# abalakrishna123/recovery-rl

Measured on AMD Instinct MI355X. Metric: env-steps/sec + SAC grad-steps/sec, Navigation1 4096 envs, 1/2/4/8 GPU, higher is better.
Workload: dtype f32

## Files before the change

### include/rrl_hip.h

```cpp
#ifndef RRL_HIP_H
#define RRL_HIP_H

#include <stdint.h>

#ifdef __cplusplus
extern "C" {
#endif

#define RRL_OK 0
#define RRL_EINVAL (-1)
#define RRL_ELAUNCH (-2)
#define RRL_ECAPTURE (-5)
#define RRL_EPLANS (-6)
#define RRL_ERANGE (-3)

enum { RRL_ENV_NAV1 = 0, RRL_ENV_NAV2 = 1, RRL_ENV_MAZE = 2 };

enum {
    RRL_STREAM_STEP = 0,
    RRL_STREAM_RESET = 1,
    RRL_STREAM_OFFLINE = 2,
    RRL_STREAM_SAMPLE = 3,
    RRL_STREAM_SAMPLE_NEG = 4,
    RRL_STREAM_CEM = 5,
// ... 301 lines not shown
int rrl_adam_step_multi(int n_seg, const rrl_adam_seg_t* segs, float lr, float beta1, float beta2, float eps,
                        void* stream);
#define RRL_ADAM_MAX_DUALS 4
typedef struct {
    float *log_p, *exp_avg, *exp_avg_sq, *step;
    float* value;
    const float* stat;
    float eps_safe;
    float lr;
    const float* loss_in;
    float* loss_out;
    float f_loss;
} rrl_dual_t;
int rrl_adam_step_multi_duals(int n_seg, const rrl_adam_seg_t* segs, int n_dual, const rrl_dual_t* duals, float lr,
                              float beta1, float beta2, float eps, void* stream);
int rrl_w2_pack(int G, int H, const float* W2, float* W2p, void* stream);
int rrl_normal_fill(long long n_pairs, uint64_t seed, uint64_t counter, uint64_t* counter_dev, uint64_t counter_inc,
                    float* out, void* stream);
int rrl_recovery_select(int N, const float* z, float eps_safe, const float* task_action, int ld_task,
                        const float* rec_action, float* real_action, uint8_t* recovery, float* task_out,
                        void* stream);

#define RRL_EPLOG_I32 6
typedef struct {
    int32_t* rec_i32;
    double* rec_f64;
    int64_t cap;
    int64_t* state;
} rrl_episode_log_t;

int rrl_episode_log_append(int64_t n, const float* reward, const uint8_t* constraint, const uint8_t* success,
                           const uint8_t* ep_done, const uint8_t* recovery, int32_t* ep_len, double* ep_ret,
                           int32_t* ep_viol, int32_t* ep_rec, const rrl_episode_log_t* log, void* stream);

typedef struct {
    int hq, he, n_nets;
    const float *q_w1, *q_b1, *q_w2, *q_b2, *q_w3, *q_b3;
    const float *e_w0, *e_b0, *e_w1, *e_b1, *e_w2, *e_b2, *e_w3, *e_b3;
    const float *inputs_mu, *inputs_sigma, *max_logvar, *min_logvar;
} rrl_plan_weights_t;

int rrl_plan_supported(int hq, int he, int n_nets, int npart, int d_obs, int d_act);
long long rrl_plan_pack_floats(int hq, int he, int n_nets);
long long rrl_plan_scratch_floats(int n_nets, long long M, int pop);
int rrl_plan_pack(const rrl_plan_weights_t* w, int f16x3, float* packed, void* stream);
typedef struct {
    const float* packed;
    int hq, he, n_nets, npart;
    int f16x3;
    long long M;
    const int32_t* m_dev;
    int pop, plan_hor;
    const float *cur_obs, *ac_seqs, *noise;
    uint64_t seed, counter;
    uint64_t* counter_dev;
    uint64_t counter_inc;
    float *scratch, *costs;
} rrl_plan_cost_t;
int rrl_plan_cost(const rrl_plan_cost_t* a, void* stream);

typedef struct {
    int n_nets, d_in, hidden, d_out;
    float *w0, *b0, *w1, *b1, *w2, *b2, *w3, *b3, *max_logvar, *min_logvar;
    const float *mu, *sigma;
    float *g_w0, *g_b0, *g_w1, *g_b1, *g_w2, *g_b2, *g_w3, *g_b3, *g_max_logvar, *g_min_logvar, *g_logvar_part;
    float *g2_w0, *g2_b0, *g2_w1, *g2_b1, *g2_w2, *g2_b2, *g2_w3, *g2_b3;
// ... 166 lines not shown
```

### recovery_rl_amd/_lib.py

```python
import ctypes as C
import os
import subprocess

_HERE = os.path.dirname(os.path.abspath(__file__))
CSRC = os.path.join(_HERE, "csrc")
SO_PATH = os.environ.get("RRL_HIP_LIB") or os.path.join(CSRC, "librrl_hip.so")
INCLUDE = os.path.join(os.path.dirname(_HERE), "include")

HIP_SOURCES = ["nav_kernels.hip", "replay_kernels.hip", "maze_kernels.hip", "cem_kernels.hip",
               "mlp_kernels.hip", "mlp_fwd_kernels.hip", "update_kernels.hip", "log_kernels.hip", "plan_kernels.hip", "ens_train_kernels.hip",
               "ens_train_big_kernels.hip", "sqrl_kernels.hip", "qsample_kernels.hip", "eval_kernels.hip"]
HIPCC_FLAGS = ["--offload-arch=gfx950", "-O3", "-std=c++17", "-fPIC", "-shared",
               "-ffp-contract=off", "-Wall", "-Wno-unused-function",
               "-Wno-bitwise-instead-of-logical"]

SOURCE_FLAGS = {
    "nav_kernels.hip": ["-mllvm", "-amdgpu-atomic-optimizer-strategy=None"],
    "maze_kernels.hip": ["-mllvm", "-amdgpu-atomic-optimizer-strategy=None"],
    "update_kernels.hip": ["-mllvm", "-amdgpu-atomic-optimizer-strategy=None"],
}

EXPORTS = [
    "rrl_abi_version", "rrl_last_hip_error", "rrl_counter_add",
    "rrl_nav_step", "rrl_nav_step_compact", "rrl_nav_reset", "rrl_nav_rollout", "rrl_nav_offline_rollouts",
    "rrl_nav_offline",
    "rrl_maze_step", "rrl_maze_reset", "rrl_maze_offline",
    "rrl_replay_push", "rrl_sample_multi", "rrl_draw_select", "rrl_mlp3_forward_riders",
    "rrl_nav_step_push_x", "rrl_maze_step_push_x",
    "rrl_sample_multi_packed", "rrl_pack_clear", "rrl_mlp3_forward_multi_packed", "rrl_mlp_head_backward_multi_packed",
    "rrl_mlp_hidden_backward_multi_packed", "rrl_mlp_backward_pair_multi_packed", "rrl_adam_step_multi_packed", "rrl_nav_step_push_packed",
    "rrl_maze_step_push_packed",
    "rrl_adam_step_multi_duals_packed", "rrl_rcpo_penalty_packed", "rrl_policy_heads_fwd_multi_packed",
    "rrl_cem_sample", "rrl_cem_update", "rrl_cem_begin", "rrl_cem_finish",
    "rrl_gemm_f32", "rrl_mlp3_forward", "rrl_mlp3_is_split",
    "rrl_mlp3_forward_multi", "rrl_mlp_head_backward_multi", "rrl_mlp_hidden_backward_multi",
    "rrl_mlp_input_backward_multi", "rrl_mlp_backward_pair_multi", "rrl_policy_heads_fwd_multi",
    "rrl_loss_dout", "rrl_rcpo_penalty", "rrl_adam_step_multi_duals",
    "rrl_adam_step_multi", "rrl_w2_pack", "rrl_normal_fill", "rrl_recovery_select", "rrl_episode_log_append",
    "rrl_plan_supported", "rrl_plan_pack_floats", "rrl_plan_scratch_floats", "rrl_plan_pack", "rrl_plan_cost",
    "rrl_ens_train_supported", "rrl_ens_scratch_floats", "rrl_ens_train_grad", "rrl_ens_train_epoch",
    "rrl_ens_train_big_supported", "rrl_ens_big_scratch_floats", "rrl_ens_train_grad_big", "rrl_ens_train_epoch_big",
    "rrl_sqrl_scratch_floats", "rrl_sqrl_act", "rrl_sqrl_act_packed",
    "rrl_qsample_scratch_floats", "rrl_qsample_act", "rrl_qsample_act_gated", "rrl_qsample_act_packed",
    "rrl_eval_rollout", "rrl_eval_rollout_packed", "rrl_eval_rollout_maze", "rrl_eval_rollout_maze_packed",
    "rrl_eval_rollout_qs", "rrl_eval_rollout_qs_packed",
    "rrl_eval_rollout_sqrl", "rrl_eval_rollout_sqrl_packed",
]

class RRLError(RuntimeError):
    pass


def _sources():
    return [os.path.join(CSRC, f) for f in HIP_SOURCES if os.path.exists(os.path.join(CSRC, f))]


def _stale():
    if not os.path.exists(SO_PATH):
        return True
    t = os.path.getmtime(SO_PATH)
    deps = _sources() + [os.path.join(CSRC, f) for f in os.listdir(CSRC) if f.endswith(".hpp")]
    deps.append(os.path.join(INCLUDE, "rrl_hip.h"))
    return any(os.path.getmtime(d) > t for d in deps)


_FLAG_PROBES = {}


def flags_supported(hipcc, flags):
    key = (hipcc,) + tuple(flags)
    if key not in _FLAG_PROBES:
# ... 25 lines not shown
        extra = SOURCE_FLAGS.get(os.path.basename(src), [])
        if extra and not flags_supported(hipcc, extra):
            extra = []
        cmd = [hipcc] + compile_flags + extra + ["-I", INCLUDE, "-c", "-o", obj, src]
        if verbose:
            print(" ".join(cmd))
        subprocess.check_call(cmd)
        return obj

    with ThreadPoolExecutor(max_workers=jobs or min(4, os.cpu_count() or 1)) as pool:
        objs = list(pool.map(compile_one, _sources()))
    cmd = [hipcc, "--offload-arch=gfx950", "-fPIC", "-shared", "-o", SO_PATH] + objs
    if verbose:
        print(" ".join(cmd))
    subprocess.check_call(cmd)
    return SO_PATH


class rrl_replay_t(C.Structure):
    _fields_ = [("s", C.c_void_p), ("a", C.c_void_p), ("r", C.c_void_p), ("s2", C.c_void_p),
                ("m", C.c_void_p), ("cap", C.c_int64), ("state", C.c_void_p),
                ("pos_cnt", C.c_void_p), ("flags", C.c_int32), ("pinned", C.c_int64)]


REPLAY_CLAMP_STRATIFIED = 1
DRAW_UNIFORM, DRAW_STRATIFIED, DRAW_DEMO_SHARE = 0, 1, 2


class rrl_episode_log_t(C.Structure):
    _fields_ = [("rec_i32", C.c_void_p), ("rec_f64", C.c_void_p), ("cap", C.c_int64), ("state", C.c_void_p)]


EPLOG_I32 = 6
ADAM_MAX_SEGS = 12
LOSS_SAC_CRITIC, LOSS_SAC_POLICY, LOSS_QRISK_CRITIC, LOSS_QRISK_POLICY, LOSS_GAUSS_HEAD, LOSS_STOCH_HEAD, LOSS_DGD_QRISK = range(7)
ADAM_MAX_DUALS = 4


class rrl_ens_t(C.Structure):
    _fields_ = [("n_nets", C.c_int), ("d_in", C.c_int), ("hidden", C.c_int), ("d_out", C.c_int)] + [
        (name, C.c_void_p) for name in ("w0", "b0", "w1", "b1", "w2", "b2", "w3", "b3", "max_logvar", "min_logvar",
                                        "mu", "sigma", "g_w0", "g_b0", "g_w1", "g_b1", "g_w2", "g_b2", "g_w3", "g_b3",
                                        "g_max_logvar", "g_min_logvar", "g_logvar_part", "g2_w0", "g2_b0", "g2_w1",
                                        "g2_b1", "g2_w2", "g2_b2", "g2_w3", "g2_b3", "loss_part")]


class rrl_loss_t(C.Structure):
    _fields_ = [("kind", C.c_int), ("n_part", C.c_int), ("part_stride", C.c_longlong), ("out", C.c_void_p),
                ("out_t", C.c_void_p), ("v0", C.c_void_p), ("v1", C.c_void_p), ("v2", C.c_void_p),
                ("v3", C.c_void_p), ("alpha", C.c_void_p), ("f0", C.c_float), ("ld", C.c_int),
                ("n_heads", C.c_int), ("head_stride", C.c_longlong), ("d_action", C.c_void_p),
                ("loss", C.c_void_p), ("da_parts", C.c_int), ("da_part_stride", C.c_longlong), ("da_group", C.c_int)]


HEAD_GAUSS, HEAD_STOCH = 0, 1


class rrl_policy_head_t(C.Structure):
    _fields_ = [("kind", C.c_int), ("B", C.c_int), ("head", C.c_void_p), ("n_part", C.c_int),
                ("part_stride", C.c_longlong), ("eps", C.c_void_p), ("scale", C.c_void_p), ("bias", C.c_void_p),
                ("action", C.c_void_p), ("ld_action", C.c_int), ("logp", C.c_void_p), ("mean_out", C.c_void_p),
                ("obs_in", C.c_void_p), ("obs_out", C.c_void_p), ("log_std", C.c_void_p), ("min_log_std", C.c_float)]


class rrl_step_push_t(C.Structure):
    _fields_ = [("n", C.c_int64), ("pos", C.c_void_p), ("t", C.c_void_p), ("status", C.c_void_p), ("obs", C.c_void_p),
# ... 232 lines not shown
        "rrl_normal_fill": (ci, [ll, u64, u64, vp, u64, vp, vp]),
        "rrl_recovery_select": (ci, [ci, vp, f32, vp, ci, vp, vp, vp, vp, vp]),
        "rrl_plan_supported": (ci, [ci, ci, ci, ci, ci, ci]),
        "rrl_plan_pack_floats": (ll, [ci, ci, ci]),
        "rrl_plan_scratch_floats": (ll, [ci, ll, ci]),
        "rrl_plan_pack": (ci, [C.POINTER(rrl_plan_weights_t), ci, vp, vp]),
        "rrl_plan_cost": (ci, [C.POINTER(rrl_plan_cost_t), vp]),
        "rrl_ens_train_supported": (ci, [ci, ci, ci, ci]),
        "rrl_ens_scratch_floats": (ll, [ci]),
        "rrl_ens_train_epoch": (ci, [C.POINTER(rrl_ens_t), ci, C.POINTER(rrl_adam_seg_t), f32, f32, f32, f32, vp, vp,
                                     vp, ll, ll, ci, vp, vp, vp]),
        "rrl_ens_train_grad": (ci, [C.POINTER(rrl_ens_t), ci, vp, vp, vp, ll, vp, vp, vp]),
        "rrl_ens_train_big_supported": (ci, [ci, ci, ci]),
        "rrl_ens_big_scratch_floats": (ll, [ci, ll]),
        "rrl_ens_train_grad_big": (ci, [C.POINTER(rrl_ens_t), ll, vp, vp, vp, ll, vp, vp, vp]),
        "rrl_ens_train_epoch_big": (ci, [C.POINTER(rrl_ens_t), ci, C.POINTER(rrl_adam_seg_t), f32, f32, f32, f32, vp, vp,
                                         vp, ll, ll, ll, vp, vp, vp]),
        "rrl_sqrl_scratch_floats": (ll, [ll, ci]),
        "rrl_sqrl_act": (ci, [C.POINTER(rrl_sqrl_act_t), vp]),
        "rrl_sqrl_act_packed": (ci, [ci, C.POINTER(rrl_sqrl_act_t), vp]),
        "rrl_qsample_scratch_floats": (ll, [ll, ci]),
        "rrl_qsample_act": (ci, [C.POINTER(rrl_qsample_act_t), vp]),
        "rrl_qsample_act_gated": (ci, [C.POINTER(rrl_qsample_act_t), C.POINTER(rrl_qsample_gate_t), vp]),
        "rrl_qsample_act_packed": (ci, [ci, C.POINTER(rrl_qsample_act_t), C.POINTER(rrl_qsample_gate_t), vp]),
        "rrl_eval_rollout": (ci, [C.POINTER(rrl_eval_rollout_t), vp]),
        "rrl_eval_rollout_packed": (ci, [ci, C.POINTER(rrl_eval_rollout_t), vp]),
        "rrl_eval_rollout_maze": (ci, [C.POINTER(rrl_eval_rollout_t), ci, vp]),
        "rrl_eval_rollout_maze_packed": (ci, [ci, C.POINTER(rrl_eval_rollout_t), C.POINTER(ci), vp]),
        "rrl_eval_rollout_qs": (ci, [C.POINTER(rrl_eval_rollout_qs_t), vp]),
        "rrl_eval_rollout_qs_packed": (ci, [ci, C.POINTER(rrl_eval_rollout_qs_t), vp]),
        "rrl_eval_rollout_sqrl": (ci, [C.POINTER(rrl_eval_rollout_sqrl_t), vp]),
        "rrl_eval_rollout_sqrl_packed": (ci, [ci, C.POINTER(rrl_eval_rollout_sqrl_t), vp]),
        "rrl_episode_log_append": (ci, [i64, vp, vp, vp, vp, vp, vp, vp, vp, vp, C.POINTER(rrl_episode_log_t), vp]),
    }
    for name, (res, args) in sig.items():
        fn = getattr(lib, name)
        fn.restype = res
        fn.argtypes = args
    for name in EXPORTS:
        if name not in sig:
            getattr(lib, name)


def load():
    global _lib
    if _lib is not None:
        return _lib
    import torch
    if not os.path.exists(SO_PATH):
        raise RRLError(
            "librrl_hip.so is not built (%s). Run `python -c 'import __graft_entry__ as g; "
            "g.build()'`; there is no CPU fallback for the hot path." % SO_PATH)
    lib = C.CDLL(SO_PATH)
    _declare(lib)
    _lib = lib
    return lib


_RC_TEXT = {-1: "invalid argument", -2: "launch failed", -3: "size out of range",
            -5: "a packed launch met a new argument block while the stream was capturing (launch it once before the capture)",
            -6: "too many distinct argument blocks of packed launches alive (rrl_pack_clear)"}


def check(rc, what):
    if rc != 0:
        lib = load()
# ... 24 lines not shown
```

### recovery_rl_amd/checkpoint.py

```python
import os
import random

import numpy as np
import torch

from .fast_update import FLAT_NETS as _FLAT_NETS

FORMAT = 1

_ENV_FIELDS = ("pos", "t", "obs", "prev_obs", "next_obs", "reward", "action_clipped", "_flags", "tick")
_DUALS = ("alpha", "nu", "lambda_RCPO")


def _cpu(t):
    return t.detach().to("cpu", copy=True)


def replay_state(mem):
    size = int(mem.state[1].item())
    out = {"capacity": mem.capacity, "size": size, "state": _cpu(mem.state), "tick": _cpu(mem.tick),
           "len": mem._len, "len_exact": mem._len_exact, "pinned": mem.pinned}
    for name in ("s", "a", "r", "s2", "m"):
        out[name] = _cpu(getattr(mem, name)[:size])
    if mem.pos_cnt is not None:
# ... 115 lines not shown

def loop_state(loop):
    out = {"stats": _cpu(loop.stats), "reward_sums": _cpu(loop.reward_sums), "ep_reward": _cpu(loop.ep_reward),
           "total_numsteps": loop.total_numsteps, "updates": loop.updates, "host_updates": list(loop.host_updates),
           "num_constraint_violations": loop.num_constraint_violations}
    if getattr(loop, "sqrl_hip", False):
        out["sqrl_tick"] = _cpu(loop.sqrl_actor().sqrl_tick)
    if getattr(loop, "qsample_hip", False):
        out["qsample_tick"] = _cpu(loop.qsample_actor().qsample_tick)
    log = loop.episode_log
    if log is not None:
        out["episode_log"] = {"ep_len": _cpu(log.ep_len), "ep_ret": _cpu(log.ep_ret), "ep_viol": _cpu(log.ep_viol),
                              "ep_rec": _cpu(log.ep_rec), "state": _cpu(log.state),
                              "rec_i32": _cpu(log.rec_i32[:int(log.state[0].item())]),
                              "rec_f64": _cpu(log.rec_f64[:int(log.state[0].item())])}
    return out


def load_loop_state(loop, sd):
    loop.stats.copy_(sd["stats"])
    loop.reward_sums.copy_(sd["reward_sums"])
    loop.ep_reward.copy_(sd["ep_reward"])
    loop.total_numsteps, loop.updates = sd["total_numsteps"], sd["updates"]
    loop.host_updates = list(sd["host_updates"])
    loop.num_constraint_violations = sd["num_constraint_violations"]
    loop.obs = loop.env.obs
    loop.graph = None
    if "sqrl_tick" in sd:
        loop.sqrl_actor().sqrl_tick.copy_(sd["sqrl_tick"])
    if "qsample_tick" in sd:
        loop.qsample_actor().qsample_tick.copy_(sd["qsample_tick"])
    if loop.episode_log is not None and "episode_log" in sd:
        log, e = loop.episode_log, sd["episode_log"]
        for f in ("ep_len", "ep_ret", "ep_viol", "ep_rec", "state"):
            getattr(log, f).copy_(e[f])
        k = e["rec_i32"].shape[0]
        log.rec_i32[:k].copy_(e["rec_i32"])
        log.rec_f64[:k].copy_(e["rec_f64"])


def mpc_state(mpc):
    return {"model": {n: _cpu(v) for n, v in mpc.model.state_dict().items()},
            "optim": mpc.model.optim.state_dict() if hasattr(mpc.model, "optim") else None,
            "trainer": mpc._trainer.state_dict() if mpc._trainer is not None else None,
            "train_in": _cpu(mpc.train_in), "train_targs": _cpu(mpc.train_targs),
            "has_been_trained": mpc.has_been_trained, "prev_sol": _cpu(mpc.prev_sol),
            "cem_tick": _cpu(mpc.optimizer.tick)}


def load_mpc_state(mpc, sd):
    mpc.model.load_state_dict(sd["model"])
    if sd["optim"] is not None:
        mpc.model.optim.load_state_dict(sd["optim"])
    if sd.get("trainer") is not None:
        from .ensemble_train import FusedEnsembleTrainer
        if mpc._trainer is None:
            mpc._trainer = FusedEnsembleTrainer(mpc.model, lr=mpc.model.optim.param_groups[0]["lr"])
        mpc._trainer.load_state_dict(sd["trainer"])
    dev = mpc.device
    mpc.train_in, mpc.train_targs = sd["train_in"].to(dev), sd["train_targs"].to(dev)
    mpc.has_been_trained = sd["has_been_trained"]
    mpc.prev_sol.copy_(sd["prev_sol"])
    mpc.optimizer.tick.copy_(sd["cem_tick"])


def experiment_state(exp, extra=None):
# ... 73 lines not shown
```

### recovery_rl_amd/csrc/log_kernels.hip

```cpp
#include "rrl_host.hpp"

using namespace rrl_host;

namespace {

__global__ __launch_bounds__(kBlock) void episode_log_kernel(
    int64_t n, const float* __restrict__ reward, const uint8_t* __restrict__ constraint,
    const uint8_t* __restrict__ success, const uint8_t* __restrict__ ep_done,
    const uint8_t* __restrict__ recovery, int32_t* __restrict__ ep_len, double* __restrict__ ep_ret,
    int32_t* __restrict__ ep_viol, int32_t* __restrict__ ep_rec, int32_t* __restrict__ rec_i32,
    double* __restrict__ rec_f64, int64_t cap, int64_t* __restrict__ state) {
    const int64_t iteration = state[1];
    const int64_t stride = (int64_t)gridDim.x * blockDim.x;
    const int64_t n_iter = (n + stride - 1) / stride;
    for (int64_t it = 0; it < n_iter; ++it) {
        const int64_t i = it * stride + blockIdx.x * (int64_t)blockDim.x + threadIdx.x;
        const bool live = i < n;
        float r = 0.f;
        int c = 0, rec = 0, len = 0, viol = 0, recs = 0;
        double ret = 0.0;
        bool finished = false;
        if (live) {
            r = reward[i];
            c = constraint[i] != 0;
// ... 12 lines not shown
            base = __shfl(base, leader, 64);
            if (finished) {
                const long long slot = base + __popcll(bal & ((1ULL << lane) - 1ULL));
                if (slot < cap) {
                    int32_t* ri = rec_i32 + slot * RRL_EPLOG_I32;
                    ri[0] = (int32_t)i;
                    ri[1] = (int32_t)iteration;
                    ri[2] = len;
                    ri[3] = viol;
                    ri[4] = recs;
                    ri[5] = (success[i] ? 1 : 0) | (c ? 2 : 0) | (rec ? 4 : 0);
                    rec_f64[slot * 2 + 0] = ret;
                    rec_f64[slot * 2 + 1] = (double)r;
                }
            }
        }
        if (live) {
            ep_len[i] = finished ? 0 : len;
            ep_ret[i] = finished ? 0.0 : ret;
            ep_viol[i] = finished ? 0 : viol;
            ep_rec[i] = finished ? 0 : recs;
        }
    }
    __syncthreads();
    if (threadIdx.x == 0) {
        const unsigned long long ticket = atomicAdd((unsigned long long*)&state[2], 1ULL);
        if (ticket == gridDim.x - 1) {
            state[1] = iteration + 1;
            state[2] = 0;
        }
    }
}

}

extern "C" {

int rrl_episode_log_append(int64_t n, const float* reward, const uint8_t* constraint, const uint8_t* success,
                           const uint8_t* ep_done, const uint8_t* recovery, int32_t* ep_len, double* ep_ret,
                           int32_t* ep_viol, int32_t* ep_rec, const rrl_episode_log_t* log, void* stream) {
    if (!reward || !constraint || !success || !ep_done || !ep_len || !ep_ret || !ep_viol || !ep_rec || !log ||
        !log->rec_i32 || !log->rec_f64 || !log->state || log->cap <= 0 || n <= 0)
        return RRL_EINVAL;
    hipLaunchKernelGGL(episode_log_kernel, dim3(grid_for(n)), dim3(kBlock), 0, (hipStream_t)stream, n, reward,
                       constraint, success, ep_done, recovery, ep_len, ep_ret, ep_viol, ep_rec, log->rec_i32,
                       log->rec_f64, log->cap, log->state);
    return check_launch();
}

}
```

### recovery_rl_amd/episode_log.py

```python
import ctypes as C

import numpy as np
import torch

from . import _lib

EPISODE_DTYPE = np.dtype([("env", "<i4"), ("iteration", "<i4"), ("length", "<i4"), ("constraint_steps", "<i4"),
                          ("recovery_steps", "<i4"), ("flags", "<i4"), ("ret", "<f8"), ("last_reward", "<f8")])
FLAG_SUCCESS, FLAG_CONSTRAINT, FLAG_RECOVERY = 1, 2, 4


class EpisodeLog:

    def __init__(self, num_envs, capacity, device):
        dev = _lib.require_gpu(device)
        self.lib = _lib.load()
        self.n, self.capacity, self.device = int(num_envs), int(capacity), dev
        self.ep_len = torch.zeros(self.n, dtype=torch.int32, device=dev)
        self.ep_ret = torch.zeros(self.n, dtype=torch.float64, device=dev)
        self.ep_viol = torch.zeros(self.n, dtype=torch.int32, device=dev)
        self.ep_rec = torch.zeros(self.n, dtype=torch.int32, device=dev)
        self.rec_i32 = torch.zeros(self.capacity, _lib.EPLOG_I32, dtype=torch.int32, device=dev)
        self.rec_f64 = torch.zeros(self.capacity, 2, dtype=torch.float64, device=dev)
        self.state = torch.zeros(3, dtype=torch.int64, device=dev)
        self._desc = _lib.rrl_episode_log_t(self.rec_i32.data_ptr(), self.rec_f64.data_ptr(), self.capacity,
                                            self.state.data_ptr())

    def append(self, reward, constraint, success, ep_done, recovery=None):
        if recovery is not None and recovery.dtype != torch.uint8:
            recovery = recovery.to(torch.uint8)
        args = (self.n, _lib.ptr(reward), _lib.ptr(constraint), _lib.ptr(success), _lib.ptr(ep_done),
                _lib.ptr(recovery), _lib.ptr(self.ep_len), _lib.ptr(self.ep_ret), _lib.ptr(self.ep_viol),
                _lib.ptr(self.ep_rec), C.byref(self._desc))
        from .fast_update import record
        record("call", self.lib.rrl_episode_log_append, args, (reward, constraint, success, ep_done, recovery, self))
        _lib.check(self.lib.rrl_episode_log_append(*args, _lib.current_stream()), "rrl_episode_log_append")

    def attach(self, a):
        p = _lib.ptr
        a.log_rec_i32, a.log_rec_f64, a.log_cap, a.log_state = p(self.rec_i32), p(self.rec_f64), self.capacity, p(self.state)
        a.log_len, a.log_ret, a.log_viol, a.log_rec = p(self.ep_len), p(self.ep_ret), p(self.ep_viol), p(self.ep_rec)

    def drain(self):
        count = int(self.state[0].item())
        if count > self.capacity:
            raise _lib.RRLError("episode log overflow: %d records for capacity %d (drain more often)"
                                % (count, self.capacity))
        out = np.zeros(count, dtype=EPISODE_DTYPE)
        if count:
            ri, rf = self.rec_i32[:count], self.rec_f64[:count]
            order = torch.argsort(ri[:, 1].to(torch.int64) * (1 << 32) + ri[:, 0].to(torch.int64))
            ri, rf = ri[order].cpu().numpy(), rf[order].cpu().numpy()
            for k, name in enumerate(("env", "iteration", "length", "constraint_steps", "recovery_steps", "flags")):
                out[name] = ri[:, k]
            out["ret"], out["last_reward"] = rf[:, 0], rf[:, 1]
        self.state[0].zero_()
        return out


class InfoRing:
    FIELDS = 11

    def __init__(self, k, steps, device, action_high, mid_episode=False):
        self.k, self.steps, self.device = int(k), int(steps), device
        self.partial = [bool(mid_episode)] * int(k)
        self.rows = torch.zeros(self.steps, self.k, self.FIELDS, dtype=torch.float32, device=device)
        self.state = torch.zeros(self.k, 2, dtype=torch.float32, device=device)
        self.filled = 0
        self.hi = float(action_high)
        self.open = [[] for _ in range(self.k)]

    def before_step(self, obs):
        self.state.copy_(obs[:self.k])

    def after_step(self, env, real_action, recovery):
        if self.filled >= self.steps:
# ... 83 lines not shown
```

### recovery_rl_amd/experiment.py

```python
import datetime
import itertools
import os
import os.path as osp
import pickle
import time

import numpy as np
import torch

from . import distributed as dist_utils
from .env import make_env, make_vec_env, register_env
from .replay_memory import ConstraintReplayMemory, ReplayMemory
from .sac import SAC
from .fused import mlp3_supported
from .utils import linear_schedule, trace_range

STAT_KEYS = ("env_steps", "episodes", "num_viols", "viol_and_recovery", "viol_and_no_recovery",
             "num_successes", "recovery_steps", "constraint_steps", "sac_updates", "qrisk_updates")


def uses_constraint_buffer(cfg):
    return cfg.use_recovery or cfg.DGD_constraints or cfg.RCPO


# ... 326 lines not shown
        self.graph = g
        self._graph_out = (self.obs, self._last_recovery, self._last_real_action)
        self.graph_many, self.graph_many_iters = None, max(1, int(iters if iters is not None else
                                                                   getattr(self.cfg, "graph_iterations", 4)))
        if self.graph_many_iters > 1:
            self.graph_many = record(self.graph_many_iters)
            restore()
            self._graph_many_out = (self.obs, self._last_recovery, self._last_real_action)
            self.obs, self._last_recovery, self._last_real_action = self._graph_out
        return warmup

    def replay(self):
        if getattr(self.env, "_status_live", None) != self._graph_status_live:
            raise RuntimeError("the env's live state representation changed since the graph was captured "
                               "(status word live: %r at capture, %r now); capture again"
                               % (self._graph_status_live, getattr(self.env, "_status_live", None)))
        if self._eager_for_keys():
            return self.vector_step(True, False, self._graph_online_qrisk)
        self.graph.replay()
        self.obs, self._last_recovery, self._last_real_action = self._graph_out
        self._advance_mirrors(1)
        return self.obs

    def _eager_for_keys(self):
        ahead = getattr(self.memory, "ahead", None)
        if ahead is None:
            return False
        if not self._graph_ahead:
            ahead.drop()
            return False
        return not ahead.ready(self.cfg.batch_size)

    def _advance_mirrors(self, iterations):
        self.total_numsteps += self.n * iterations
        self.host_updates[0] += self._graph_updates[0] * iterations
        self.host_updates[1] += self._graph_updates[1] * iterations
        self.updates += self.cfg.updates_per_step * iterations
        self.agent.safety_critic.updates += self._graph_updates[1] * iterations
        for mem, rows in zip((self.memory, self.recovery_memory), self._graph_rows):
            mem._len = min(mem._len + rows * iterations, mem.capacity)
        if self.cfg.add_both_transitions:
            self.memory._len_exact = False

    def advance(self, iterations):
        k = self.graph_many_iters if self.graph_many is not None else 0
        if iterations > 0 and self._eager_for_keys():
            self.vector_step(True, False, self._graph_online_qrisk)
            iterations -= 1
        while k > 1 and iterations >= k:
            if getattr(self.env, "_status_live", None) != self._graph_status_live:
                break
            self.graph_many.replay()
            self.obs, self._last_recovery, self._last_real_action = self._graph_many_out
            self._advance_mirrors(k)
            iterations -= k
        for _ in range(iterations):
            self.replay()
        return self.obs

    def read_stats(self):
        mems = [m for m in (self.memory, self.recovery_memory) if hasattr(m, "state") and torch.is_tensor(m.state)]
        if len(mems) == 2 and self.stats.is_cuda:
            packed = torch.cat([self.stats.to(torch.int64), mems[0].state[3:4], mems[1].state[3:4],
                                self.reward_sums.view(torch.int64)]).cpu()
            n = self.stats.numel()
            for m, code in zip(mems, packed[n:n + 2].tolist()):
                if code:
                    m.check_error()
            vals = packed[:n].tolist()
            sums = packed[n + 2:].view(torch.float64).tolist()
        else:
            self.memory.check_error()
            self.recovery_memory.check_error()
            vals = self.stats.cpu().tolist()
            sums = self.reward_sums.cpu().tolist()
        vals[8], vals[9] = self.host_updates
        out = dict(zip(STAT_KEYS, vals))
        out["reward_sum"], out["episode_return_sum"] = float(sums[0]), float(sums[1])
        return out


MAX_COVER_ROWS = 1 << 28
ROW_BYTES = 32


def cover_rows_limit(device=None, seeds_per_gpu=1):
    limit = MAX_COVER_ROWS
    if device is not None and torch.cuda.is_available() and torch.device(device).type == "cuda":
        total = torch.cuda.get_device_properties(torch.device(device)).total_memory
        limit = min(limit, int(total // 8 // max(int(seeds_per_gpu), 1) // ROW_BYTES))
    return limit


def replay_capacities(cfg, device=None):
    cap, safe_cap = int(cfg.replay_size), int(cfg.safe_replay_size)
    n = int(getattr(cfg, "num_envs", 1))
    if n <= 1 or getattr(cfg, "keep_replay_size", False) or cfg.num_steps <= min(cap, safe_cap):
        return cap, safe_cap
# ... 721 lines not shown
```

### recovery_rl_amd/packed.py

```python
import ctypes as C
import os

import torch

from . import _lib
from . import fast_update
from .fast_update import FLAT_NETS


class PackedLoop:
    MAX_SEEDS = 16
    PAIR_MAX_SEEDS = int(os.environ.get("RRL_PACK_PAIR_BLOCK_MAX_SEEDS", "8"))

    FRAG_MAX_SEEDS = 8

    def __init__(self, loops, online_qrisk=True):
        if not 1 <= len(loops) <= self.MAX_SEEDS:
            raise ValueError("1 .. %d seeds per GPU" % self.MAX_SEEDS)
        self.loops = list(loops)
        self.S = len(loops)
        if self.S > self.FRAG_MAX_SEEDS and any(getattr(loop, "sqrl_hip", False) for loop in self.loops):
            raise ValueError("SQRL's constraint-sampling acting pass (rrl_sqrl_act_packed) packs at most %d seeds per GPU: it "
                             "reads the fragment-order W2 copy of Q_risk, which packed runs keep up to that many seeds only "
                             "(got %d)" % (self.FRAG_MAX_SEEDS, self.S))
# ... 107 lines not shown
        return stages

    @property
    def launches(self):
        total = 0
        for fn, args, ops in self.stages:
            if ops[0][0] == "pair_bwd":
                kinds = {op[1][k].loss.kind for op in ops for k in range(op[3])}
                one = (_lib.LOSS_SAC_CRITIC, _lib.LOSS_SAC_POLICY, _lib.LOSS_QRISK_CRITIC, _lib.LOSS_QRISK_POLICY, _lib.LOSS_DGD_QRISK)
                outputs = {1 if kind in one else kind for kind in kinds}
                total += 1 if min(kinds) >= 0 and len(outputs) == 1 and self.S <= self.PAIR_MAX_SEEDS else 2
            elif ops[0][0] == "call":
                total += len(ops)
            else:
                total += 1
        return total

    @staticmethod
    def _call_each(calls, stream):
        for fn, args in calls:
            rc = fn(*args, stream)
            if rc:
                return rc
        return 0

    def launch(self):
        st = _lib.current_stream()
        for fn, args, _ in self.stages:
            _lib.check(fn(*args, st), getattr(fn, "__name__", "packed stage"))

    def _advance_host_mirrors(self, iterations=1):
        for loop in self.loops:
            cfg = loop.cfg
            loop.total_numsteps += loop.n * iterations
            loop.host_updates[0] += cfg.updates_per_step * iterations
            loop.updates += cfg.updates_per_step * iterations
            if self.online_qrisk:
                loop.host_updates[1] += cfg.updates_per_step * iterations
                loop.agent.safety_critic.updates += cfg.updates_per_step * iterations
            from .experiment import uses_constraint_buffer
            for mem, rows in ((loop.memory, loop.n), (loop.recovery_memory, loop.n if uses_constraint_buffer(cfg) else 0)):
                mem._len = min(mem._len + rows * iterations, mem.capacity)

    def step(self):
        self.launch()
        self._advance_host_mirrors()

    def capture(self, warmup=2, settle=2, around=None, iters=None):
        def real(fn):
            if around is not None:
                around[0]()
            fn()
            if around is not None:
                around[1]()

        def settle_once():
            for loop in self.loops:
                loop.vector_step(True, False, self.online_qrisk)
        for _ in range(settle):
            real(settle_once)
        real(self.record)
        dev = self.loops[0].device
        side = torch.cuda.Stream(device=dev)
        side.wait_stream(torch.cuda.current_stream(dev))
        with torch.cuda.stream(side):
            for _ in range(max(warmup, 1)):
# ... 40 lines not shown
```

Baseline: 29.36 million.

## Drain episode log on GPU with bitmap sort and fused stats readback

Adds a multi-kernel episode-log drain that orders records by (iteration, env) using a bitmap, a prefix scan and a scatter, then writes them with a header into a pinned host buffer. Stats words are copied in the same pass, so read_stats and drain share one device-to-host transfer instead of separate torch gathers and copies. The aim is to cut host-side sorting and synchronisation at log boundaries. It adds five kernel launches, including a single-block scan, a prepared-state cache that must be invalidated on every step, and a fallback to the torch path when keys are invalid.

```diff
diff --git a/include/rrl_hip.h b/include/rrl_hip.h
--- a/include/rrl_hip.h
+++ b/include/rrl_hip.h
@@ -357,6 +357,28 @@
 int rrl_episode_log_append(int64_t n, const float* reward, const uint8_t* constraint, const uint8_t* success,
                            const uint8_t* ep_done, const uint8_t* recovery, int32_t* ep_len, double* ep_ret,
                            int32_t* ep_viol, int32_t* ep_rec, const rrl_episode_log_t* log, void* stream);
+
+#define RRL_LOG_DRAIN_HEADER 4
+#define RRL_EPLOG_RECORD_BYTES 40
+#define RRL_LOG_DRAIN_MAX_SRC 4
+#define RRL_LOG_DRAIN_META 8
+#define RRL_LOG_DRAIN_WORK_WORDS(span, n_envs) (RRL_LOG_DRAIN_META + 2 * (int64_t)(span) * (((int64_t)(n_envs) + 63) / 64))
+enum { RRL_LOG_DRAIN_OK = 0, RRL_LOG_DRAIN_OVERFLOW = 1, RRL_LOG_DRAIN_NOFIT = 2, RRL_LOG_DRAIN_KEYS = 3 };
+enum { RRL_LOG_DRAIN_RESET = 1, RRL_LOG_DRAIN_RESET_ONLY = 2 };
+typedef struct {
+    const rrl_episode_log_t* log;
+    int64_t n_envs;
+    int32_t flags;
+    int32_t n_src;
+    const void* src[RRL_LOG_DRAIN_MAX_SRC];
+    int64_t src_words[RRL_LOG_DRAIN_MAX_SRC];
+    uint64_t* work;
+    int64_t work_words;
+    int32_t* order;
+    void* out;
+    int64_t out_records;
+} rrl_log_drain_t;
+int rrl_episode_log_drain(const rrl_log_drain_t* a, void* stream);
 
 typedef struct {
     int hq, he, n_nets;
diff --git a/recovery_rl_amd/_lib.py b/recovery_rl_amd/_lib.py
--- a/recovery_rl_amd/_lib.py
+++ b/recovery_rl_amd/_lib.py
@@ -37,6 +37,7 @@
     "rrl_mlp_input_backward_multi", "rrl_mlp_backward_pair_multi", "rrl_policy_heads_fwd_multi",
     "rrl_loss_dout", "rrl_rcpo_penalty", "rrl_adam_step_multi_duals",
     "rrl_adam_step_multi", "rrl_w2_pack", "rrl_normal_fill", "rrl_recovery_select", "rrl_episode_log_append",
+    "rrl_episode_log_drain",
     "rrl_plan_supported", "rrl_plan_pack_floats", "rrl_plan_scratch_floats", "rrl_plan_pack", "rrl_plan_cost",
     "rrl_ens_train_supported", "rrl_ens_scratch_floats", "rrl_ens_train_grad", "rrl_ens_train_epoch",
     "rrl_ens_train_big_supported", "rrl_ens_big_scratch_floats", "rrl_ens_train_grad_big", "rrl_ens_train_epoch_big",
@@ -128,6 +129,26 @@
 
 
 EPLOG_I32 = 6
+LOG_DRAIN_HEADER, LOG_DRAIN_MAX_SRC, LOG_DRAIN_META, EPLOG_RECORD_BYTES = 4, 4, 8, 40
+LOG_DRAIN_OK, LOG_DRAIN_OVERFLOW, LOG_DRAIN_NOFIT, LOG_DRAIN_KEYS = range(4)
+LOG_DRAIN_RESET, LOG_DRAIN_RESET_ONLY = 1, 2
+
+
+class rrl_log_drain_t(C.Structure):
+    _fields_ = [("log", C.POINTER(rrl_episode_log_t)), ("n_envs", C.c_int64), ("flags", C.c_int32), ("n_src", C.c_int32),
+                ("src", C.c_void_p * LOG_DRAIN_MAX_SRC), ("src_words", C.c_int64 * LOG_DRAIN_MAX_SRC),
+                ("work", C.c_void_p), ("work_words", C.c_int64), ("order", C.c_void_p), ("out", C.c_void_p),
+                ("out_records", C.c_int64)]
+
+
+def log_drain_work_words(span, n_envs):
+    return LOG_DRAIN_META + 2 * int(span) * ((int(n_envs) + 63) // 64)
+
+
+def log_drain_fits(span, n_envs, work_words):
+    return int(span) * ((int(n_envs) + 63) // 64) <= (int(work_words) - LOG_DRAIN_META) // 2
+
+
 ADAM_MAX_SEGS = 12
 LOSS_SAC_CRITIC, LOSS_SAC_POLICY, LOSS_QRISK_CRITIC, LOSS_QRISK_POLICY, LOSS_GAUSS_HEAD, LOSS_STOCH_HEAD, LOSS_DGD_QRISK = range(7)
 ADAM_MAX_DUALS = 4
@@ -426,6 +447,7 @@
         "rrl_eval_rollout_sqrl": (ci, [C.POINTER(rrl_eval_rollout_sqrl_t), vp]),
         "rrl_eval_rollout_sqrl_packed": (ci, [ci, C.POINTER(rrl_eval_rollout_sqrl_t), vp]),
         "rrl_episode_log_append": (ci, [i64, vp, vp, vp, vp, vp, vp, vp, vp, vp, C.POINTER(rrl_episode_log_t), vp]),
+        "rrl_episode_log_drain": (ci, [C.POINTER(rrl_log_drain_t), vp]),
     }
     for name, (res, args) in sig.items():
         fn = getattr(lib, name)
diff --git a/recovery_rl_amd/checkpoint.py b/recovery_rl_amd/checkpoint.py
--- a/recovery_rl_amd/checkpoint.py
+++ b/recovery_rl_amd/checkpoint.py
@@ -171,6 +171,7 @@
         loop.qsample_actor().qsample_tick.copy_(sd["qsample_tick"])
     if loop.episode_log is not None and "episode_log" in sd:
         log, e = loop.episode_log, sd["episode_log"]
+        log.invalidate()
         for f in ("ep_len", "ep_ret", "ep_viol", "ep_rec", "state"):
             getattr(log, f).copy_(e[f])
         k = e["rec_i32"].shape[0]
diff --git a/recovery_rl_amd/csrc/log_kernels.hip b/recovery_rl_amd/csrc/log_kernels.hip
--- a/recovery_rl_amd/csrc/log_kernels.hip
+++ b/recovery_rl_amd/csrc/log_kernels.hip
@@ -68,6 +68,152 @@
     }
 }
 
+struct DrainJob {
+    const int32_t* rec_i32;
+    const double* rec_f64;
+    int64_t cap;
+    int64_t* state;
+    int64_t n_envs, words;
+    int32_t flags, n_src;
+    const uint64_t* src[RRL_LOG_DRAIN_MAX_SRC];
+    int64_t src_words[RRL_LOG_DRAIN_MAX_SRC];
+    int64_t* meta;
+    uint64_t* bitmap;
+    uint64_t* prefix;
+    int64_t bitmap_words;
+    int32_t* order;
+    uint64_t* out;
+    int64_t out_records, src_total;
+};
+
+constexpr int kScanBlock = 1024;
+
+__device__ __forceinline__ void drain_flag(int64_t* meta, int status) {
+    atomicMax((unsigned long long*)&meta[1], (unsigned long long)status);
+}
+
+__global__ __launch_bounds__(kBlock) void drain_begin_kernel(DrainJob j) {
+    const int64_t stride = (int64_t)gridDim.x * blockDim.x;
+    for (int64_t w = blockIdx.x * (int64_t)blockDim.x + threadIdx.x; w < j.bitmap_words; w += stride) j.bitmap[w] = 0;
+    if (blockIdx.x != 0) return;
+    int64_t off = 0;
+    for (int s = 0; s < j.n_src; ++s) {
+        for (int64_t w = threadIdx.x; w < j.src_words[s]; w += blockDim.x) j.out[off + w] = j.src[s][w];
+        off += j.src_words[s];
+    }
+    if (threadIdx.x == 0) {
+        const int64_t count = j.state[0];
+        int64_t status = RRL_LOG_DRAIN_OK;
+        if (count > j.cap) status = RRL_LOG_DRAIN_OVERFLOW;
+        else if (count < 0) status = RRL_LOG_DRAIN_KEYS;
+        else if (count > j.out_records) status = RRL_LOG_DRAIN_NOFIT;
+        const bool some = status == RRL_LOG_DRAIN_OK && count > 0;
+        const int64_t lo = some ? j.rec_i32[1] : 0, hi = some ? j.rec_i32[(count - 1) * RRL_EPLOG_I32 + 1] : 0;
+        if (some && hi < lo) status = RRL_LOG_DRAIN_KEYS;
+        j.meta[0] = count;
+        j.meta[1] = status;
+        j.meta[2] = lo;
+        j.meta[3] = hi;
+        if (status != RRL_LOG_DRAIN_OK) {
+            uint64_t* h = j.out + j.src_total;
+            h[0] = (uint64_t)count;
+            h[1] = (uint64_t)status;
+            h[2] = 0;
+            h[3] = 0;
+        }
+    }
+}
+
+__global__ __launch_bounds__(kBlock) void drain_mark_kernel(DrainJob j) {
+    const int64_t count = j.meta[0];
+    if (j.meta[1] != RRL_LOG_DRAIN_OK || count == 0) return;
+    const int64_t lo = j.meta[2], span = j.meta[3] - lo + 1;
+    const int64_t stride = (int64_t)gridDim.x * blockDim.x, first = blockIdx.x * (int64_t)blockDim.x + threadIdx.x;
+    if (span > j.bitmap_words / j.words) {
+        if (first == 0) drain_flag(j.meta, RRL_LOG_DRAIN_NOFIT);
+        return;
+    }
+    for (int64_t s = first; s < count; s += stride) {
+        const int64_t env = j.rec_i32[s * RRL_EPLOG_I32], it = j.rec_i32[s * RRL_EPLOG_I32 + 1];
+        if (env < 0 || env >= j.n_envs || it < lo || it > j.meta[3]) {
+            drain_flag(j.meta, RRL_LOG_DRAIN_KEYS);
+            continue;
+        }
+        const unsigned long long bit = 1ULL << (env & 63);
+        const unsigned long long old = atomicOr((unsigned long long*)&j.bitmap[(it - lo) * j.words + (env >> 6)], bit);
+        if (old & bit) drain_flag(j.meta, RRL_LOG_DRAIN_KEYS);
+    }
+}
+
+__global__ __launch_bounds__(kScanBlock) void drain_scan_kernel(DrainJob j) {
+    __shared__ int64_t part[kScanBlock];
+    const int64_t count = j.meta[0];
+    int64_t status = j.meta[1];
+    const int t = threadIdx.x;
+    if (status == RRL_LOG_DRAIN_OVERFLOW) return;
+    const bool live = status == RRL_LOG_DRAIN_OK && count > 0;
+    if (live) {
+        const int64_t nw = (j.meta[3] - j.meta[2] + 1) * j.words;
+        const int64_t per = (nw + kScanBlock - 1) / kScanBlock;
+        const int64_t w0 = t * per < nw ? t * per : nw, w1 = w0 + per < nw ? w0 + per : nw;
+        int64_t mine = 0;
+        for (int64_t w = w0; w < w1; ++w) mine += __popcll(j.bitmap[w]);
+        part[t] = mine;
+        __syncthreads();
+        for (int d = 1; d < kScanBlock; d <<= 1) {
+            const int64_t v = t >= d ? part[t - d] : 0;
+            __syncthreads();
+            part[t] += v;
+            __syncthreads();
+        }
+        int64_t run = part[t] - mine;
+        for (int64_t w = w0; w < w1; ++w) {
+            j.prefix[w] = (uint64_t)run;
+            run += __popcll(j.bitmap[w]);
+        }
+        if (part[kScanBlock - 1] != count) status = RRL_LOG_DRAIN_KEYS;
+    }
+    if (t == 0) {
+        j.meta[1] = status;
+        uint64_t* h = j.out + j.src_total;
+        h[0] = (uint64_t)count;
+        h[1] = (uint64_t)status;
+        h[2] = (uint64_t)(live ? j.meta[2] : 0);
+        h[3] = (uint64_t)(live ? j.meta[3] : 0);
+        if (status == RRL_LOG_DRAIN_OK && (j.flags & RRL_LOG_DRAIN_RESET)) j.state[0] = 0;
+    }
+}
+
+__global__ __launch_bounds__(kBlock) void drain_place_kernel(DrainJob j) {
+    const int64_t count = j.meta[0];
+    if (j.meta[1] != RRL_LOG_DRAIN_OK) return;
+    const int64_t lo = j.meta[2];
+    const int64_t stride = (int64_t)gridDim.x * blockDim.x;
+    for (int64_t s = blockIdx.x * (int64_t)blockDim.x + threadIdx.x; s < count; s += stride) {
+        const int64_t env = j.rec_i32[s * RRL_EPLOG_I32], it = j.rec_i32[s * RRL_EPLOG_I32 + 1];
+        const int64_t w = (it - lo) * j.words + (env >> 6);
+        const int64_t place = (int64_t)j.prefix[w] + __popcll(j.bitmap[w] & ((1ULL << (env & 63)) - 1ULL));
+        if (place < count) j.order[place] = (int32_t)s;
+    }
+}
+
+__global__ __launch_bounds__(kBlock) void drain_copy_kernel(DrainJob j) {
+    const int64_t count = j.meta[0];
+    if (j.meta[1] != RRL_LOG_DRAIN_OK) return;
+    constexpr int kWords = RRL_EPLOG_RECORD_BYTES / 8, kIntWords = RRL_EPLOG_I32 / 2;
+    const uint64_t* ri = (const uint64_t*)j.rec_i32;
+    const uint64_t* rf = (const uint64_t*)j.rec_f64;
+    uint64_t* out = j.out + j.src_total + RRL_LOG_DRAIN_HEADER;
+    const int64_t stride = (int64_t)gridDim.x * blockDim.x;
+    for (int64_t i = blockIdx.x * (int64_t)blockDim.x + threadIdx.x; i < count * kWords; i += stride) {
+        const int64_t s = j.order[i / kWords];
+        const int k = (int)(i % kWords);
+        out[i] = k < kIntWords ? ri[s * kIntWords + k] : rf[s * 2 + (k - kIntWords)];
+    }
+}
+
+__global__ void drain_reset_kernel(int64_t* state) { state[0] = 0; }
+
 }
 
 extern "C" {
@@ -84,4 +230,52 @@
     return check_launch();
 }
 
-}
+int rrl_episode_log_drain(const rrl_log_drain_t* a, void* stream) {
+    if (!a || !a->log || !a->log->state) return RRL_EINVAL;
+    hipStream_t st = (hipStream_t)stream;
+    if (a->flags & RRL_LOG_DRAIN_RESET_ONLY) {
+        hipLaunchKernelGGL(drain_reset_kernel, dim3(1), dim3(1), 0, st, a->log->state);
+        return check_launch();
+    }
+    const rrl_episode_log_t* log = a->log;
+    if (!log->rec_i32 || !log->rec_f64 || log->cap <= 0 || a->n_envs <= 0 || !a->work || !a->order || !a->out ||
+        a->out_records < 0 || a->n_src < 0 || a->n_src > RRL_LOG_DRAIN_MAX_SRC)
+        return RRL_EINVAL;
+    if (log->cap > INT32_MAX || a->n_envs > INT32_MAX) return RRL_ERANGE;
+    DrainJob j;
+    j.rec_i32 = log->rec_i32;
+    j.rec_f64 = log->rec_f64;
+    j.cap = log->cap;
+    j.state = log->state;
+    j.n_envs = a->n_envs;
+    j.words = (a->n_envs + 63) / 64;
+    j.flags = a->flags;
+    j.n_src = a->n_src;
+    j.src_total = 0;
+    for (int s = 0; s < RRL_LOG_DRAIN_MAX_SRC; ++s) {
+        const bool used = s < a->n_src;
+        if (used && (a->src_words[s] < 0 || a->src_words[s] > 64 || (a->src_words[s] > 0 && !a->src[s]))) return RRL_EINVAL;
+        j.src[s] = used ? (const uint64_t*)a->src[s] : nullptr;
+        j.src_words[s] = used ? a->src_words[s] : 0;
+        j.src_total += j.src_words[s];
+    }
+    j.bitmap_words = (a->work_words - RRL_LOG_DRAIN_META) / 2;
+    if (j.bitmap_words < j.words) return RRL_EINVAL;
+    j.meta = (int64_t*)a->work;
+    j.bitmap = a->work + RRL_LOG_DRAIN_META;
+    j.prefix = j.bitmap + j.bitmap_words;
+    j.order = a->order;
+    j.out = (uint64_t*)a->out;
+    j.out_records = a->out_records;
+    const int64_t reach = log->cap < a->out_records ? log->cap : a->out_records;
+    const int g_rec = grid_for(reach) < 256 ? grid_for(reach) : 256;
+    const int g_copy = grid_for(reach * (RRL_EPLOG_RECORD_BYTES / 8)) < 256 ? grid_for(reach * (RRL_EPLOG_RECORD_BYTES / 8)) : 256;
+    hipLaunchKernelGGL(drain_begin_kernel, dim3(grid_for(j.bitmap_words) < 64 ? grid_for(j.bitmap_words) : 64), dim3(kBlock), 0, st, j);
+    hipLaunchKernelGGL(drain_mark_kernel, dim3(g_rec), dim3(kBlock), 0, st, j);
+    hipLaunchKernelGGL(drain_scan_kernel, dim3(1), dim3(kScanBlock), 0, st, j);
+    hipLaunchKernelGGL(drain_place_kernel, dim3(g_rec), dim3(kBlock), 0, st, j);
+    hipLaunchKernelGGL(drain_copy_kernel, dim3(g_copy), dim3(kBlock), 0, st, j);
+    return check_launch();
+}
+
+}
diff --git a/recovery_rl_amd/episode_log.py b/recovery_rl_amd/episode_log.py
--- a/recovery_rl_amd/episode_log.py
+++ b/recovery_rl_amd/episode_log.py
@@ -1,4 +1,5 @@
 import ctypes as C
+import os
 
 import numpy as np
 import torch
@@ -12,7 +13,7 @@
 
 class EpisodeLog:
 
-    def __init__(self, num_envs, capacity, device):
+    def __init__(self, num_envs, capacity, device, drain_span=None):
         dev = _lib.require_gpu(device)
         self.lib = _lib.load()
         self.n, self.capacity, self.device = int(num_envs), int(capacity), dev
@@ -25,10 +26,15 @@
         self.state = torch.zeros(3, dtype=torch.int64, device=dev)
         self._desc = _lib.rrl_episode_log_t(self.rec_i32.data_ptr(), self.rec_f64.data_ptr(), self.capacity,
                                             self.state.data_ptr())
+        self.drain_span = int(drain_span) if drain_span is not None else -(-self.capacity // self.n) + 1
+        self.last_path = None
+        self._drain_bufs = None
+        self._prepared = None
 
     def append(self, reward, constraint, success, ep_done, recovery=None):
         if recovery is not None and recovery.dtype != torch.uint8:
             recovery = recovery.to(torch.uint8)
+        self._prepared = None
         args = (self.n, _lib.ptr(reward), _lib.ptr(constraint), _lib.ptr(success), _lib.ptr(ep_done),
                 _lib.ptr(recovery), _lib.ptr(self.ep_len), _lib.ptr(self.ep_ret), _lib.ptr(self.ep_viol),
                 _lib.ptr(self.ep_rec), C.byref(self._desc))
@@ -37,11 +43,83 @@
         _lib.check(self.lib.rrl_episode_log_append(*args, _lib.current_stream()), "rrl_episode_log_append")
 
     def attach(self, a):
+        self._prepared = None
         p = _lib.ptr
         a.log_rec_i32, a.log_rec_f64, a.log_cap, a.log_state = p(self.rec_i32), p(self.rec_f64), self.capacity, p(self.state)
         a.log_len, a.log_ret, a.log_viol, a.log_rec = p(self.ep_len), p(self.ep_ret), p(self.ep_viol), p(self.ep_rec)
 
+    def invalidate(self):
+        self._prepared = None
+
+    @staticmethod
+    def kernel_drain_enabled():
+        return os.environ.get("RRL_LOG_DRAIN", "1") != "0"
+
+    def _buffers(self):
+        if self._drain_bufs is None:
+            words = _lib.log_drain_work_words(self.drain_span, self.n)
+            work = torch.zeros(words, dtype=torch.int64, device=self.device)
+            order = torch.zeros(max(self.capacity, 1), dtype=torch.int32, device=self.device)
+            head = 8 * (_lib.LOG_DRAIN_MAX_SRC * 64 + _lib.LOG_DRAIN_HEADER)
+            out = torch.empty(head + self.capacity * _lib.EPLOG_RECORD_BYTES, dtype=torch.uint8, pin_memory=True)
+            self._drain_bufs = (work, order, out, out.numpy())
+        return self._drain_bufs
+
+    def _drain_call(self, flags, sources=()):
+        work, order, out, out_np = self._buffers()
+        a = _lib.rrl_log_drain_t()
+        a.log, a.n_envs, a.flags, a.n_src = C.pointer(self._desc), self.n, flags, len(sources)
+        for k, (p, w) in enumerate(sources):
+            a.src[k], a.src_words[k] = p, w
+        a.work, a.work_words, a.order = work.data_ptr(), work.numel(), order.data_ptr()
+        a.out, a.out_records = out.data_ptr(), self.capacity
+        n_src = sum(w for _, w in sources)
+        head = out_np[8 * n_src:8 * (n_src + _lib.LOG_DRAIN_HEADER)].view(np.int64)
+        head[0] = -1
+        _lib.check(self.lib.rrl_episode_log_drain(C.byref(a), _lib.current_stream()), "rrl_episode_log_drain")
+        torch.cuda.current_stream(self.device).synchronize()
+        count, status = int(head[0]), int(head[1])
+        if count < 0:
+            raise _lib.RRLError("rrl_episode_log_drain left its header unwritten")
+        words = out_np[:8 * n_src].view(np.int64).copy()
+        vals, at = [], 0
+        for _, w in sources:
+            vals.append(words[at:at + w])
+            at += w
+        rec = None
+        if status == _lib.LOG_DRAIN_OK:
+            at = 8 * (n_src + _lib.LOG_DRAIN_HEADER)
+            rec = out_np[at:at + count * EPISODE_DTYPE.itemsize].copy().view(EPISODE_DTYPE)
+        return vals, status, count, rec
+
+    def prepare(self, sources):
+        vals, status, count, rec = self._drain_call(0, sources)
+        self._prepared = (status, count, rec)
+        return vals
+
     def drain(self):
+        if not self.kernel_drain_enabled():
+            self._prepared = None
+            return self._drain_torch()
+        prepared, self._prepared = self._prepared, None
+        if prepared is None:
+            status, count, rec = self._drain_call(_lib.LOG_DRAIN_RESET)[1:]
+        else:
+            status, count, rec = prepared
+            if status == _lib.LOG_DRAIN_OK:
+                a = _lib.rrl_log_drain_t()
+                a.log, a.flags = C.pointer(self._desc), _lib.LOG_DRAIN_RESET_ONLY
+                _lib.check(self.lib.rrl_episode_log_drain(C.byref(a), _lib.current_stream()), "rrl_episode_log_drain")
+        if status == _lib.LOG_DRAIN_OVERFLOW:
+            raise _lib.RRLError("episode log overflow: %d records for capacity %d (drain more often)"
+                                % (count, self.capacity))
+        if status != _lib.LOG_DRAIN_OK:
+            return self._drain_torch()
+        self.last_path = "kernel"
+        return rec
+
+    def _drain_torch(self):
+        self.last_path = "torch"
         count = int(self.state[0].item())
         if count > self.capacity:
             raise _lib.RRLError("episode log overflow: %d records for capacity %d (drain more often)"
diff --git a/recovery_rl_amd/experiment.py b/recovery_rl_amd/experiment.py
--- a/recovery_rl_amd/experiment.py
+++ b/recovery_rl_amd/experiment.py
@@ -382,6 +382,8 @@
         return not ahead.ready(self.cfg.batch_size)
 
     def _advance_mirrors(self, iterations):
+        if self.episode_log is not None:
+            self.episode_log.invalidate()
         self.total_numsteps += self.n * iterations
         self.host_updates[0] += self._graph_updates[0] * iterations
         self.host_updates[1] += self._graph_updates[1] * iterations
@@ -410,10 +412,16 @@
 
     def read_stats(self):
         mems = [m for m in (self.memory, self.recovery_memory) if hasattr(m, "state") and torch.is_tensor(m.state)]
+        log = self.episode_log
         if len(mems) == 2 and self.stats.is_cuda:
-            packed = torch.cat([self.stats.to(torch.int64), mems[0].state[3:4], mems[1].state[3:4],
-                                self.reward_sums.view(torch.int64)]).cpu()
             n = self.stats.numel()
+            if log is not None and log.kernel_drain_enabled() and self.stats.dtype == torch.int64:
+                words = log.prepare([(self.stats.data_ptr(), n), (mems[0].state.data_ptr() + 24, 1),
+                                     (mems[1].state.data_ptr() + 24, 1), (self.reward_sums.data_ptr(), 2)])
+                packed = torch.from_numpy(np.concatenate(words))
+            else:
+                packed = torch.cat([self.stats.to(torch.int64), mems[0].state[3:4], mems[1].state[3:4],
+                                    self.reward_sums.view(torch.int64)]).cpu()
             for m, code in zip(mems, packed[n:n + 2].tolist()):
                 if code:
                     m.check_error()
diff --git a/recovery_rl_amd/packed.py b/recovery_rl_amd/packed.py
--- a/recovery_rl_amd/packed.py
+++ b/recovery_rl_amd/packed.py
@@ -163,6 +163,8 @@
     def _advance_host_mirrors(self, iterations=1):
         for loop in self.loops:
             cfg = loop.cfg
+            if loop.episode_log is not None:
+                loop.episode_log.invalidate()
             loop.total_numsteps += loop.n * iterations
             loop.host_updates[0] += cfg.updates_per_step * iterations
             loop.updates += cfg.updates_per_step * iterations
```

Result: no change. 29.64 million (median of 6 runs) (+1.0%).
